# timoblak/sq-recovery

Hardware: NVIDIA B200
Metric: fused SQ implicit-loss fwd+bwd throughput (higher is better)
Workload: dtype f32

## Files before the change

sq_recovery_b200/csrc/sqloss.cu:

```cuda
#include <cuda_runtime.h>
#include <stdint.h>
#include <stdio.h>
#include <string.h>
#include <new>

#include "../../include/sqloss.h"
#ifdef SQ_TIMELINE
__device__ unsigned long long g_bwd_stats[2];
#endif
#if defined(SQ_TIMELINE) && defined(SQ_BWD_STATS)
#define SQ_BWD_HOOK(a) do { const unsigned m_ = __ballot_sync(0xffffffffu, (a)); if ((threadIdx.x & 31) == 0) { \
    atomicAdd(&g_bwd_stats[0], 1ull); atomicAdd(&g_bwd_stats[1], (unsigned long long)__popc(m_)); } } while (0)
#endif
#ifdef SQ_ITEMLOG
__device__ float g_planlog[4 * 65536];
__device__ int g_itemlog[4 * 65536];
#endif
#ifdef SQ_COUNT
__device__ unsigned long long g_count[8];
#define SQ_COUNT_HOOK(i, n) do { if ((threadIdx.x & 31) == 0) atomicAdd(&g_count[i], (unsigned long long)(n)); } while (0)
#else
#define SQ_COUNT_HOOK(i, n) do { } while (0)
#endif
#include "sq_core.cuh"
// ... 123 lines not shown
#define SQ_CLASSES 32
#endif
constexpr int kClasses = SQ_CLASSES;
static_assert(kClasses >= 4 && kClasses <= 32, "the class counters live in one warp's lanes and in the 256-byte control block");
#ifndef SQ_PLAN_THREADS
#define SQ_PLAN_THREADS 512
#endif
constexpr int kPlanThreads = SQ_PLAN_THREADS;
constexpr int kPlanThreadsSmall = 128;
constexpr int kPlanMaxItems = 8192;

struct Control {
    unsigned int ticket;
    unsigned int cursor;
    unsigned int retired;
    unsigned int pad0;
    unsigned int qcount[kClasses];
    unsigned int pad1[64 - 4 - kClasses];
};
static_assert(sizeof(Control) == 256, "Control block is 256 bytes");

constexpr int kRow = 20;
struct Scratch {
    Control* ctl;
    SampleFull* pred;
    SampleFull* tru;
    float* partials;
    double* per_sample;
    double* tv_sum;
    unsigned long long* counts;
    unsigned char* item_class;
    int* queue;
    int queue_cap;
};

inline size_t align_up(size_t v, size_t a) { return (v + a - 1) / a * a; }

size_t scratch_layout(int batch, int n, char* base, Scratch* s) {
    const Layout L = make_layout(n > 0 ? n : 1, 1);
    size_t off = 0;
    auto take = [&](size_t bytes) { size_t o = off; off = align_up(off + bytes, 256); return o; };
    const size_t o_ctl = take(sizeof(Control));
    const size_t o_pred = take(sizeof(SampleFull) * (size_t)batch);
    const size_t o_true = take(sizeof(SampleFull) * (size_t)batch);
    size_t rows_ps = (size_t)L.rows_per_sample;
    const size_t lsq_rows = (size_t)(L.slots + kThreads - 1) / kThreads;
    if (lsq_rows > rows_ps) rows_ps = lsq_rows;
    const size_t o_part = take(sizeof(float) * kRow * rows_ps * (size_t)batch);
    const size_t o_ps = take(sizeof(double) * (size_t)batch);
    const size_t o_tv = take(sizeof(double) * (size_t)batch);
    const size_t o_cnt = take(sizeof(unsigned long long) * 2 * (size_t)batch);
    const size_t cap = (size_t)L.rows_per_sample * (size_t)batch;
    const bool queued = L.rows_per_sample <= kPlanMaxItems && cap < (1u << 30);
    const size_t o_queue = take(queued ? sizeof(int) * kClasses * cap : 0);
    const size_t o_cls = take(queued ? cap : 0);
    if (s) {
        s->ctl = reinterpret_cast<Control*>(base + o_ctl);
        s->pred = reinterpret_cast<SampleFull*>(base + o_pred);
        s->tru = reinterpret_cast<SampleFull*>(base + o_true);
        s->partials = reinterpret_cast<float*>(base + o_part);
        s->per_sample = reinterpret_cast<double*>(base + o_ps);
        s->tv_sum = reinterpret_cast<double*>(base + o_tv);
        s->counts = reinterpret_cast<unsigned long long*>(base + o_cnt);
        s->queue = queued ? reinterpret_cast<int*>(base + o_queue) : nullptr;
        s->item_class = queued ? reinterpret_cast<unsigned char*>(base + o_cls) : nullptr;
        s->queue_cap = (int)cap;
    }
    return off;
}

__device__ __forceinline__ void pdl_wait() {
#ifdef SQ_PDL
    asm volatile("griddepcontrol.wait;" ::: "memory");
#endif
}
__device__ __forceinline__ void pdl_trigger() {
#ifdef SQ_PDL
    asm volatile("griddepcontrol.launch_dependents;");
#endif
}

#ifdef SQ_TIMELINE
__device__ unsigned long long g_plan_ts[16];
__device__ __forceinline__ unsigned long long gtime() { unsigned long long t; asm volatile("mov.u64 %0, %%globaltimer;" : "=l"(t)); return t; }
#endif
constexpr int kSampleWords = (int)(sizeof(Sample) / 4);
constexpr int kFullWords = (int)(sizeof(SampleFull) / 4);
static_assert(sizeof(Sample) % 8 == 0 && sizeof(SampleFull) % 8 == 0, "Sample records must be word-copyable");

__device__ __forceinline__ void load_params(const void* params, int dtype, int b, double* p) {
#pragma unroll
    for (int i = 0; i < 12; ++i)
        p[i] = dtype == SQ_F64 ? static_cast<const double*>(params)[12 * (size_t)b + i]
                               : (double)static_cast<const float*>(params)[12 * (size_t)b + i];
}

__global__ void __launch_bounds__(128)
prep_kernel(const void* params, int dtype, int batch, int clamp, Grid g, SampleFull* out, Control* ctl) {
    __shared__ SampleFull Ssh[4];
    const int warp = threadIdx.x >> 5, lane = threadIdx.x & 31;
    const int b = blockIdx.x * 4 + warp;
    if (blockIdx.x == 0 && threadIdx.x == 0 && ctl) { ctl->ticket = 0u; ctl->cursor = 0u; }
    if (b >= batch) return;
    if (lane == 0) {
        double p[12];
        load_params(params, dtype, b, p);
        prep_sample(p, clamp != 0, g, Ssh[warp]);
    }
    __syncwarp();
    const uint32_t* src = reinterpret_cast<const uint32_t*>(&Ssh[warp]);
    uint32_t* dst = reinterpret_cast<uint32_t*>(out + b);
    for (int w = lane; w < kFullWords; w += 32) dst[w] = src[w];
}

__device__ int group_planes(const Sample& S, const Grid& g, const Layout& L, float bound, int group, float die = 0.f) {
    float cx, cy, hx, hy;
    if (L.patched) {
        const int pw = L.n >> 3, pb = group / pw, pa = group - pb * pw;
        cx = (float)(pa << 3) + 3.5f; cy = (float)(pb << 2) + 1.5f; hx = 3.5f; hy = 1.5f;
    } else {
        xfast_group_footprint(L.n, group, cx, cy, hx, hy);
    }
    return die > 0.f ? footprint_walk(S, g, bound, die, cx, cy, hx, hy) : footprint_planes(S, g, bound, cx, cy, hx, hy);
}

template <int NS, int THREADS>
__global__ void __launch_bounds__(THREADS)
plan_kernel(const void* params_a, const void* params_b, int dtype, int clamp, int heads, Grid g, Layout L, float bound, float die,
            SampleFull* out_a, SampleFull* out_b, Control* ctl, unsigned long long* counts, int* queue, int cap,
            unsigned char* item_class, const float* __restrict__ target, long long tstride, const int* __restrict__ row_off,
            const int* __restrict__ col_off, double* tv_sum) {
    __shared__ SampleFull Ssh[NS];
    __shared__ unsigned char cls[kPlanMaxItems];
    __shared__ unsigned int ccnt[kClasses], cbase[kClasses];
    __shared__ double tv_part[THREADS / 32];
    const int b = blockIdx.x;
#ifdef SQ_TIMELINE
    unsigned long long ts[6]; int nts = 0;
#define SQ_STAMP() do { if (nts < 6) ts[nts++] = gtime(); } while (0)
#else
#define SQ_STAMP() do { } while (0)
#endif
    SQ_STAMP();
    if (threadIdx.x < kClasses) ccnt[threadIdx.x] = 0u;
    if (threadIdx.x == 64) {
        if (b == 0) { ctl->ticket = 0u; ctl->cursor = 0u; }
        if (counts) { counts[2 * b] = 0ull; counts[2 * b + 1] = 0ull; }
    }
    if ((threadIdx.x >> 5) < NS) {
        __shared__ double psh[NS][12];
        const int w = threadIdx.x >> 5, lane = threadIdx.x & 31;
        double* p = psh[w];
        const void* params = w == 0 ? params_a : params_b;
        if (lane < 12)
            p[lane] = dtype == SQ_F64 ? static_cast<const double*>(params)[12 * (size_t)b + lane]
                                      : (double)static_cast<const float*>(params)[12 * (size_t)b + lane];
        __syncwarp();
        double hp_l = 0.0, hrn = 1.0;
        if (heads) {
            double v = 0.0;
            if (lane < 8) { hp_l = (double)(float)(1.0 / (1.0 + exp(-p[lane]))); v = hp_l; }
            else if (lane < 12) {
                hrn = 1.0 / sqrt(p[8] * p[8] + p[9] * p[9] + p[10] * p[10] + p[11] * p[11]);
                v = (double)(float)(p[lane] * hrn);
// ... 26 lines not shown
            int i = t;
            for (; i + 7 * T < npix; i += 8 * T) {
                float v[8];
#pragma unroll
                for (int u = 0; u < 8; ++u) v[u] = pixel(i + u * T);
#pragma unroll
                for (int u = 0; u < 8; u += 2) { acc0 += (double)fabsf(v[u]); acc1 += (double)fabsf(v[u + 1]); }
            }
            {
                float v[8];
#pragma unroll
                for (int u = 0; u < 8; ++u) { const int iu = i + u * T; v[u] = iu < npix ? pixel(iu) : 0.f; }
#pragma unroll
                for (int u = 0; u < 8; u += 2) { acc0 += (double)fabsf(v[u]); acc1 += (double)fabsf(v[u + 1]); }
            }
            double d = acc0 + acc1;
#pragma unroll
            for (int o = 16; o > 0; o >>= 1) d += __shfl_xor_sync(0xffffffffu, d, o);
            if (lane == 0) tv_part[warp] = d;
            SQ_STAMP();
        }
    }
    __syncthreads();
    SQ_STAMP();
    if (tv_sum && threadIdx.x == 0) {
        double d = 0.0;
        for (int w = NS; w < THREADS / 32; ++w) d += tv_part[w];
        tv_sum[b] = d;
    }
    for (int w = threadIdx.x; w < NS * kFullWords; w += THREADS) {
        const int which = w / kFullWords, i = w - which * kFullWords;
        reinterpret_cast<uint32_t*>((which == 0 ? out_a : out_b) + b)[i] = reinterpret_cast<const uint32_t*>(&Ssh[which])[i];
    }
    if (!queue) return;
    const int J = L.rows_per_sample;
    const int max_cost = L.cpt * L.n * NS;
    for (int j = threadIdx.x; j < J; j += THREADS) {
        int c = kClasses - 1;
        int cost = 0;
        for (int k = 0; k < L.cpt; ++k) {
            const int group = j + k * J;
            if (group * 32 >= L.slots) break;
#pragma unroll
            for (int w = 0; w < NS; ++w) cost += group_planes(Ssh[w], g, L, bound, group, NS == 1 ? die : 0.f);
        }
        if (cost > 0) {
            if (kClasses == 8) { c = 0; while (c < kClasses - 2 && (cost << (c + 1)) <= max_cost) ++c; }
            else {
                c = (int)((float)(kClasses / 8) * __log2f((float)max_cost / (float)cost));
                c = c < 0 ? 0 : (c > kClasses - 2 ? kClasses - 2 : c);
            }
        }
#ifdef SQ_ITEMLOG
        if (NS == 1 && b * J + j < 65536) { float* lg = g_planlog + 4 * (b * J + j); lg[0] = (float)c; lg[1] = (float)cost; lg[2] = lg[3] = 0.f; }
#endif
        cls[j] = (unsigned char)c;
        if (item_class) item_class[(size_t)b * J + j] = (unsigned char)c;
        atomicAdd(&ccnt[c], 1u);
    }
    __syncthreads();
    SQ_STAMP();
    if (threadIdx.x < kClasses) {
        const unsigned int c = ccnt[threadIdx.x];
        cbase[threadIdx.x] = c ? atomicAdd(&ctl->qcount[threadIdx.x], c) : 0u;
        ccnt[threadIdx.x] = 0u;
    }
    __syncthreads();
    for (int j = threadIdx.x; j < J; j += THREADS) {
        const int c = cls[j];
        const unsigned int r = atomicAdd(&ccnt[c], 1u);
#ifdef SQ_DEBUG_BOUNDS
        if (c < 0 || c >= kClasses || cbase[c] + r >= (unsigned int)cap || b * J + j >= cap) __trap();
#endif
        queue[(size_t)c * cap + cbase[c] + r] = b * J + j;
    }
#ifdef SQ_TIMELINE
    SQ_STAMP();
    if (b == 7 && (threadIdx.x == 0 || threadIdx.x == 100)) {
        const int o = threadIdx.x == 0 ? 0 : 8;
        for (int i = 0; i < nts; ++i) g_plan_ts[o + i] = ts[i];
        g_plan_ts[o + 7] = nts;
    }
#endif
}

__device__ __forceinline__ float warp_sum(float v) {
#pragma unroll
    for (int o = 16; o > 0; o >>= 1) v += __shfl_xor_sync(0xffffffffu, v, o);
    return v;
}

// ... 94 lines not shown
            for (int w = 0; w < kWarps; ++w) s += red[w][threadIdx.x];
        }
        row[threadIdx.x] = s;
    }
}

__device__ __forceinline__ void load_sample(Sample* dst, const SampleFull* src) {
    const uint32_t* s = reinterpret_cast<const uint32_t*>(src);
    uint32_t* d = reinterpret_cast<uint32_t*>(dst);
    for (int i = threadIdx.x; i < kSampleWords; i += blockDim.x) d[i] = s[i];
}

constexpr int kSampleRegs = (kSampleWords + 31) / 32;
struct SampleFetch {
    uint32_t w[kSampleRegs];
    __device__ __forceinline__ void fetch(const SampleFull* src, int lane) {
        const uint32_t* s = reinterpret_cast<const uint32_t*>(src);
#pragma unroll
        for (int j = 0; j < kSampleRegs; ++j) {
            const int i = lane + 32 * j;
            w[j] = i < kSampleWords ? __ldg(s + i) : 0u;
        }
    }
    __device__ __forceinline__ void commit(Sample* dst, int lane) const {
        uint32_t* d = reinterpret_cast<uint32_t*>(dst);
        __syncwarp();
#pragma unroll
        for (int j = 0; j < kSampleRegs; ++j) {
            const int i = lane + 32 * j;
            if (i < kSampleWords) d[i] = w[j];
        }
        __syncwarp();
    }
};

__device__ __forceinline__ int first_position() {
    return (int)(blockIdx.x * (blockDim.x >> 5) + (threadIdx.x >> 5));
}
__device__ __forceinline__ int next_position(unsigned int* cursor, int lane) {
    int pos = 0;
    if (lane == 0) pos = (int)(atomicAdd(cursor, 1u) + gridDim.x * (blockDim.x >> 5));
    return __shfl_sync(0xffffffffu, pos, 0);
}

struct WorkMap {
    unsigned int excl;
    __device__ __forceinline__ void init(const Control* ctl, int lane) {
        const unsigned int cnt = lane < kClasses ? __ldcg(&ctl->qcount[lane]) : 0u;
        unsigned int incl = cnt;
#pragma unroll
        for (int o = 1; o < kClasses; o <<= 1) {
            const unsigned int t = __shfl_up_sync(0xffffffffu, incl, o);
            if (lane >= o) incl += t;
        }
        excl = incl - cnt;
    }
    __device__ __forceinline__ int item(const int* __restrict__ queue, int cap, int pos, int lane) const {
        if (!queue) return pos;
        const unsigned int m = __ballot_sync(0xffffffffu, lane < kClasses && (unsigned int)pos >= excl);
        const int c = 31 - __clz((int)m);
        const unsigned int start = __shfl_sync(0xffffffffu, excl, c);
#ifdef SQ_DEBUG_BOUNDS
        if (c < 0 || c >= kClasses || (unsigned int)pos - start >= (unsigned int)cap) __trap();
        const int it = __ldg(queue + (size_t)c * cap + ((unsigned int)pos - start));
        if (it < 0 || it >= cap) __trap();
        return it;
// ... 44 lines not shown
        const unsigned int warps = gridDim.x * (blockDim.x >> 5);
        const unsigned int joiners = (unsigned int)total_items < warps ? (unsigned int)total_items : warps;
        const unsigned int before = atomicAdd(&ctl->retired, 1u);
        if (before + 1u == joiners) {
            ctl->retired = 0u;
#pragma unroll
            for (int k = 0; k < kClasses; ++k) ctl->qcount[k] = 0u;
        }
    }
}

#ifdef SQ_TIMELINE
__device__ unsigned long long g_timeline[3 * 8192];
__device__ unsigned int g_classes[kClasses];
#endif
#ifdef SQ_PHASES
__device__ unsigned long long g_phase[8];
#define SQ_PH(i) do { const long long n_ = clock64(); ph[i] += n_ - ph_t; ph_t = n_; } while (0)
#else
#define SQ_PH(i) do { } while (0)
#endif

#ifndef SQ_EARLY_MARGIN
#define SQ_EARLY_MARGIN 0
#endif
constexpr size_t kImplicitBwdSmemPerWarp = (size_t)kBwdPool * 4 * sizeof(float) + 11 * 32 * sizeof(float);
static_assert(kImplicitBwdSmemPerWarp % 32 == 0, "per-warp regions stay 32-byte aligned (BwdQueue::where carries the lane in its low bits)");

template <bool BWD, int THREADS, int MINB, int CPTMAX, bool VJP = false>
__global__ void __launch_bounds__(THREADS, MINB)
implicit_kernel(const SampleFull* __restrict__ samples, Grid g, Layout L, ImplicitParams P, int total_items,
                Control* __restrict__ ctl, const int* __restrict__ queue, int cap,
                const float* __restrict__ target, long long tstride, const int* __restrict__ row_off,
                const int* __restrict__ col_off, float* __restrict__ partials, float* __restrict__ depth_out) {
    __shared__ Sample Ssh[THREADS / 32];
#if SQ_TILE_ALIAS && defined(SQ_BWD_COMPACT)
    static_assert(!BWD || CPTMAX == 1, "SQ_TILE_ALIAS needs one column group per work item");
    static_assert(4 * kBwdPool >= kRedFloats, "pool arrays too small to hold the tile");
    __shared__ __align__(16) float tiles_static[BWD ? 1 : THREADS / 32][kRedFloats];
#else
    __shared__ __align__(16) float tiles_static[THREADS / 32][kRedFloats];
#endif
#ifdef SQ_BWD_COMPACT
    constexpr int kQN = kBwdPool;
    extern __shared__ __align__(32) unsigned char dyn_smem[];
    float* const qbuf = reinterpret_cast<float*>(dyn_smem + (size_t)(threadIdx.x >> 5) * kImplicitBwdSmemPerWarp);
    float* const colinfo_w = qbuf + 4 * kQN;
#endif
#if SQ_TILE_ALIAS && defined(SQ_BWD_COMPACT)
    float* const tile_w = BWD ? qbuf : tiles_static[threadIdx.x >> 5];
#else
    float* const tile_w = tiles_static[threadIdx.x >> 5];
#endif
    static_assert(!VJP || BWD, "the VJP mode is a mode of the fwd+bwd kernel");
    const int warp = threadIdx.x >> 5, lane = threadIdx.x & 31;
    Sample& S = Ssh[warp];
#if defined(SQ_BWD_COMPACT) && !defined(SQ_TABLES_GLOBAL)
    __shared__ __align__(16) double tabs[BWD ? 384 : 130];
    constexpr int kTabRegs = (384 + THREADS - 1) / THREADS;
    double tab_reg[kTabRegs];
    if (BWD) {
#pragma unroll
        for (int r = 0; r < kTabRegs; ++r) {
            const int i = threadIdx.x + r * THREADS;
            tab_reg[r] = i < 128 ? kExp2TabDev[i] : (i < 384 ? kLog2TabDev[i - 128] : 0.0);
        }
    }
    const RefTabs tb{tabs, tabs + 128};
#else
    const RefTabs tb = default_tabs();
#endif
    pdl_wait();
    pdl_trigger();
#ifdef SQ_TIMELINE
    const unsigned long long t_begin = gtime();
    unsigned long long t_last_fetch = t_begin, n_items = 0;
    if (BWD && blockIdx.x == 0 && threadIdx.x < kClasses) g_classes[threadIdx.x] = ctl->qcount[threadIdx.x];
#endif
    WorkPipe wp;
    wp.start(ctl, queue, cap, total_items, true, lane);
#ifdef SQ_PHASES
    long long ph[8] = {0, 0, 0, 0, 0, 0, 0, 0}, ph_t = clock64();
#endif
    {
        SampleFetch pre;
        if (wp.item >= 0) pre.fetch(samples + L.sample_of(wp.item), lane);
#if defined(SQ_BWD_COMPACT) && !defined(SQ_TABLES_GLOBAL)
        if (BWD) {
#pragma unroll
            for (int r = 0; r < kTabRegs; ++r) { const int i = threadIdx.x + r * THREADS; if (i < 384) tabs[i] = tab_reg[r]; }
            __syncthreads();
        }
#endif
        while (wp.item >= 0) {
#ifdef SQ_TIMELINE
            t_last_fetch = gtime(); ++n_items;
#endif
            int b, chunk;
            L.split(wp.item, b, chunk);
#ifdef SQ_ITEMLOG
            const long long il_t0 = clock64(); long long il_walk = 0; int il_q = 0, il_qr = 0;
#endif
            SQ_PH(7);
            pre.commit(&S, lane);
            SQ_COUNT_HOOK(4, 1);

            float loss_sum = 0.f;
            bool folded = false;
            ColIter it;
            it.init(L, chunk, lane);
            float tvs[CPTMAX];
            {
                ColIter pt = it;
#pragma unroll
                for (int k = 0; k < CPTMAX; ++k) {
                    tvs[k] = 0.f;
                    if (target && k < L.cpt) {
                        if (pt.valid(L))
                            tvs[k] = VJP ? __ldg(target + ((size_t)b * g.n + (g.n - 1 - pt.ib)) * g.n + pt.ia)
                                         : __ldg(target + (size_t)b * tstride + row_off[g.n - 1 - pt.ib] + col_off[pt.ia]);
                        pt.next(L);
                    }
                }
            }
#pragma unroll 1
            for (int k = 0; k < L.cpt; ++k) {
#ifdef SQ_EARLY_CLAIM
                if (k == L.cpt - 1 && wp.claim(lane)) pre.fetch(samples + L.sample_of(wp.next), lane);
#endif
                const int ia = it.ia, ib = it.ib;
                const bool valid = it.valid(L);
                const int row = g.n - 1 - ib, col = ia;
                it.next(L);
                float b32[3];
                column_base_f32(S, g, valid ? ia : 0, valid ? ib : 0, b32);
                int c_lo, c_hi;
                column_range(S, g, P.bound, b32, c_lo, c_hi);
                if (!valid) { c_lo = 0; c_hi = -1; }
                const int own_lo = c_hi >= c_lo ? c_lo : g.n;
                warp_range(g.n, c_lo, c_hi);
                if (c_hi < c_lo) {
#ifndef SQ_EARLY_CLAIM
                    if (k == L.cpt - 1 && wp.claim(lane)) pre.fetch(samples + L.sample_of(wp.next), lane);
#endif
                    continue;
                }
                SQ_COUNT_HOOK(5, 1);
                SQ_PH(0);
#ifdef SQ_ITEMLOG
                const long long il_w0 = clock64();
#endif
#if defined(SQ_BWD_COMPACT) && !defined(SQ_NO_STAGED_CLAIM) && !defined(SQ_EARLY_CLAIM) && SQ_EARLY_MARGIN > 0
                const bool early = BWD && k == L.cpt - 1 &&
                                   wp.item_pos + SQ_EARLY_MARGIN * (int)(gridDim.x * (THREADS / 32)) < wp.total;
                if (early) wp.claim_issue(lane);
#else
                const bool early = false;
#endif
                float bh[3], bl[3], cg[11], dxy[2];
                column_base(S, g, valid ? ia : 0, valid ? ib : 0, bh, bl, dxy);
                float depth;
#ifndef SQ_FIXHOIST
#ifdef SQ_BWD_COMPACT
                const int pool = (g.n <= kPoolMaxPlanes && S.cf0 < 1.0f) ? kQN : 0;
                float U = 0.f; int nr = 0, top = pool - 1, head = kNoLink; bool spilled = false;
                unsigned where = (unsigned)__cvta_generic_to_shared(qbuf) | (unsigned)lane;
                asm volatile("" : "+r"(where));
                const BwdQueue qwarp{qbuf, qbuf + kQN, qbuf + 2 * kQN, qbuf + 3 * kQN, pool, lane, where};
                depth = implicit_column<BWD, true, BWD>(S, g, P, bh, bl, c_lo, c_hi, own_lo, cg, &qwarp, &U, &nr, &top, &spilled, &head);
#else
                depth = implicit_column<BWD, true>(S, g, P, bh, bl, c_lo, c_hi, own_lo, cg);
#endif
#else
                if (__any_sync(0xffffffffu, column_zero_possible(S, bh)))
                    depth = implicit_column<BWD, true>(S, g, P, bh, bl, c_lo, c_hi, own_lo, cg);
                else
                    depth = implicit_column<BWD, false>(S, g, P, bh, bl, c_lo, c_hi, own_lo, cg);
#endif
                SQ_PH(1);
#ifdef SQ_ITEMLOG
                il_walk += clock64() - il_w0;
#endif
#ifndef SQ_EARLY_CLAIM
#if defined(SQ_BWD_COMPACT) && !defined(SQ_NO_STAGED_CLAIM)
                const bool staged = BWD && k == L.cpt - 1;
                if (staged) { if (!early) wp.claim_issue(lane); }
                else
#else
                const bool staged = false;
#endif
                if (k == L.cpt - 1 && wp.claim(lane)) pre.fetch(samples + L.sample_of(wp.next), lane);
#endif
#if defined(SQ_BWD_COMPACT)
                if (BWD) {
                    float wsg = 0.f;
                    float tv = tvs[0];
#pragma unroll
                    for (int q = 1; q < CPTMAX; ++q) tv = k == q ? tvs[q] : tv;
                    asm volatile("" : "+f"(tv));
                    if (valid && VJP) {
                        wsg = tv;
                    } else if (valid) {
                        if (depth_out) depth_out[((size_t)b * g.n + row) * g.n + col] = depth;
                        const float diff = depth - tv;
                        loss_sum += fabsf(diff) - fabsf(tv);
                        wsg = diff > 0.f ? 1.f : (diff < 0.f ? -1.f : 0.f);
                    }
                    const int total_r = nr, total = nr + (pool - 1 - top);
                    const bool any_spill = __any_sync(0xffffffffu, spilled && wsg != 0.f);
#ifdef SQ_ITEMLOG
                    il_q += total + (any_spill ? 1000 : 0); il_qr += total_r;
#endif
#ifndef SQ_EARLY_CLAIM
                    if (staged) {
                        wp.claim_lookup(lane);
                        if (total == 0 && wp.claim_finish()) pre.fetch(samples + L.sample_of(wp.next), lane);
                    }
#endif
                    SQ_PH(2);
                    if (total > 0 || any_spill) {
                        Acc acc;
                        float v[kRedStride];
                        if (folded) { tile_get(tile_w, v); array_to_acc(v, acc); } else acc_zero(acc);
                        if (spilled && wsg != 0.f) implicit_fold(acc, cg, wsg, dxy[0], dxy[1]);
                        if (total > 0) {
                            float* ci = colinfo_w;
                            ci[0 * 32 + lane] = bh[0]; ci[1 * 32 + lane] = bh[1]; ci[2 * 32 + lane] = bh[2];
                            ci[3 * 32 + lane] = bl[0]; ci[4 * 32 + lane] = bl[1]; ci[5 * 32 + lane] = bl[2];
                            ci[6 * 32 + lane] = wsg; ci[7 * 32 + lane] = dxy[0]; ci[8 * 32 + lane] = dxy[1];
                            ci[9 * 32 + lane] = U; ci[10 * 32 + lane] = __int_as_float(head);
                            __syncwarp();
                            SQ_COUNT_HOOK(6, total); SQ_COUNT_HOOK(7, total_r);
                            SQ_COUNT_HOOK(3, (total_r + 31) / 32); SQ_COUNT_HOOK(2, (total + 31) / 32);
                            SQ_PH(5);
                            for (int jr = lane; jr < total_r; jr += 32) {
                                const int l_ = entry_lane(qwarp.cf[jr]);
                                queue_refine_entry(S, g.step, P.kl, qwarp, jr,
                                                   f2d(ci[0 * 32 + l_]) + f2d(ci[3 * 32 + l_]), f2d(ci[1 * 32 + l_]) + f2d(ci[4 * 32 + l_]),
                                                   f2d(ci[2 * 32 + l_]) + f2d(ci[5 * 32 + l_]), tb);
                            }
                            __syncwarp();
                            SQ_PH(3);
                            const float tau = P.tl * (float)kLn2;
#ifdef SQ_DEPTH_SHIFT
                            if (!VJP && head != kNoLink) loss_sum = fmaf(wsg * tau * g.inv_n, queue_depth_shift(qwarp, head, U), loss_sum);
#endif
#ifndef SQ_EARLY_CLAIM
                            if (staged && wp.claim_finish()) pre.fetch(samples + L.sample_of(wp.next), lane);
#endif
                            auto dealt = [&](int j, Bwd& bq, float& cfq, float& dx_, float& dy_) {
                                const bool has = j < total;
                                const int at = has ? (j < total_r ? j : kQN - 1 - (j - total_r)) : 0;
                                const float tagged = has ? qwarp.cf[at] : 1.0f, x_ = has ? qwarp.x[at] : 0.0f;
                                const int l_ = entry_lane(tagged);
                                const float cf_ = entry_cf(S, tagged);
                                const float sw_ = has ? queue_suffix_weight(qwarp, at, __float_as_int(ci[10 * 32 + l_]), ci[9 * 32 + l_], tau) : 0.0f;
                                const float cbh[3] = {ci[0 * 32 + l_], ci[1 * 32 + l_], ci[2 * 32 + l_]};
                                const float cbl[3] = {ci[3 * 32 + l_], ci[4 * 32 + l_], ci[5 * 32 + l_]};
                                queue_entry_backward<true>(S, cbh, cbl, cf_, x_, sw_, ci[6 * 32 + l_], has, bq);
                                cfq = cf_; dx_ = ci[7 * 32 + l_]; dy_ = ci[8 * 32 + l_];
                            };
                            int j = lane;
#if SQ_DENSE_ILP == 2
                            for (; j - lane + 32 < total; j += 64) {
                                Bwd b0, b1; float c0, c1, x0, x1, y0, y1;
                                dealt(j, b0, c0, x0, y0);
                                dealt(j + 32, b1, c1, x1, y1);
                                acc_add_point(acc, b0, c0, x0, y0);
                                acc_add_point(acc, b1, c1, x1, y1);
                            }
#endif
                            for (; j - lane < total; j += 32) {
                                Bwd b0; float c0, x0, y0;
                                dealt(j, b0, c0, x0, y0);
                                acc_add_point(acc, b0, c0, x0, y0);
                            }
                            __syncwarp();
                            SQ_PH(4);
                        }
                        acc_to_array(acc, v);
                        v[18] = v[19] = 0.f;
// ... 490 lines not shown
    return sms[dev];
}

int persistent_blocks(int items, int warps_per_block, int min_blocks_per_sm) {
    const int need = (items + warps_per_block - 1) / warps_per_block;
    const int fill = device_sm_count() * min_blocks_per_sm;
    return need < fill ? need : fill;
}

template <auto KERNEL>
cudaError_t opt_in_dyn_smem(size_t dyn) {
    static bool opted[64] = {false};
    int dev = 0;
    cudaGetDevice(&dev);
    if (dev >= 0 && dev < 64 && !opted[dev]) {
        const cudaError_t e = cudaFuncSetAttribute(KERNEL, cudaFuncAttributeMaxDynamicSharedMemorySize, (int)dyn);
        if (e != cudaSuccess) return e;
        opted[dev] = true;
    }
    return cudaSuccess;
}

int launch_prep(const void* params, int dtype, int batch, bool clamp, const Grid& g, SampleFull* out, Control* ctl,
                cudaStream_t st) {
    if (dtype != SQ_F32 && dtype != SQ_F64) return (int)cudaErrorInvalidValue;
    prep_kernel<<<(batch + 3) / 4, 128, 0, st>>>(params, dtype, batch, clamp ? 1 : 0, g, out, ctl);
    return (int)cudaGetLastError();
}

struct PlanTarget { const float* target; long long tstride; const int* row_off; const int* col_off; };

int launch_plan(const void* params_a, const void* params_b, int dtype, int batch, bool clamp, const Grid& g,
                const Layout& L, float bound, const Scratch& s, unsigned long long* counts, unsigned char* item_class,
                const PlanTarget* pt, cudaStream_t st, bool heads = false, float die = 0.f) {
    if (dtype != SQ_F32 && dtype != SQ_F64) return (int)cudaErrorInvalidValue;
    int* queue = L.rows_per_sample <= kPlanMaxItems ? s.queue : nullptr;
    const PlanTarget none{nullptr, 0, nullptr, nullptr};
    const PlanTarget& t = pt ? *pt : none;
    const bool small = batch > 4 * device_sm_count();
    if (params_b) {
        auto k = small ? plan_kernel<2, kPlanThreadsSmall> : plan_kernel<2, kPlanThreads>;
        k<<<batch, small ? kPlanThreadsSmall : kPlanThreads, 0, st>>>(params_a, params_b, dtype, clamp ? 1 : 0, 0, g, L, bound, 0.f, s.tru, s.pred,
                                                                      s.ctl, counts, queue, s.queue_cap, queue ? item_class : nullptr,
                                                                      nullptr, 0, nullptr, nullptr, nullptr);
    } else {
        auto k = small ? plan_kernel<1, kPlanThreadsSmall> : plan_kernel<1, kPlanThreads>;
        k<<<batch, small ? kPlanThreadsSmall : kPlanThreads, 0, st>>>(params_a, nullptr, dtype, clamp ? 1 : 0, heads ? 1 : 0, g, L, bound, die, s.pred,
                                                                      nullptr, s.ctl, counts, queue, s.queue_cap, queue ? item_class : nullptr,
                                                                      t.target, t.tstride, t.row_off, t.col_off, pt ? s.tv_sum : nullptr);
    }
    return (int)cudaGetLastError();
}

}

extern "C" {

const char* sq_version(void) { return "sqloss-b200 0.1 (sm_100a)"; }

const char* sq_error_string(int err) { return cudaGetErrorString((cudaError_t)err); }

int sq_device_sm_count(int device, int* sm_count) {
    return (int)cudaDeviceGetAttribute(sm_count, cudaDevAttrMultiProcessorCount, device);
}

#ifdef SQ_COUNT
int sq_debug_counters(unsigned long long* host_out, int reset) {
    cudaError_t e = cudaMemcpyFromSymbol(host_out, g_count, sizeof(unsigned long long) * 8);
    if (e == cudaSuccess && reset) {
        const unsigned long long zero[8] = {0, 0, 0, 0, 0, 0, 0, 0};
        e = cudaMemcpyToSymbol(g_count, zero, sizeof zero);
    }
    return (int)e;
}
#endif

#ifdef SQ_ITEMLOG
int sq_debug_itemlog(float* plan_out, int* item_out, int n) {
    int rc = (int)cudaMemcpyFromSymbol(plan_out, g_planlog, sizeof(float) * 4 * (size_t)n);
    if (!rc) rc = (int)cudaMemcpyFromSymbol(item_out, g_itemlog, sizeof(int) * 4 * (size_t)n);
    return rc;
}
// ... 3 lines not shown
    int rc = (int)cudaMemcpyFromSymbol(host_out, g_phase, sizeof(unsigned long long) * 8);
    if (!rc && reset) { unsigned long long z[8] = {0, 0, 0, 0, 0, 0, 0, 0}; rc = (int)cudaMemcpyToSymbol(g_phase, z, sizeof z); }
    return rc;
}
#endif
#ifdef SQ_TIMELINE
int sq_debug_timeline(unsigned long long* host_out, int n) {
    return (int)cudaMemcpyFromSymbol(host_out, g_timeline, sizeof(unsigned long long) * 3 * (size_t)n);
}
int sq_debug_bwd(unsigned long long* host_out) {
    return (int)cudaMemcpyFromSymbol(host_out, g_bwd_stats, sizeof(unsigned long long) * 2);
}
int sq_debug_plan(unsigned long long* host_out) {
    return (int)cudaMemcpyFromSymbol(host_out, g_plan_ts, sizeof(unsigned long long) * 16);
}
int sq_debug_classes(unsigned int* host_out) {
    return (int)cudaMemcpyFromSymbol(host_out, g_classes, sizeof(unsigned int) * kClasses);
}
#endif

void sq_profile_events(void* ev_before, void* ev_after) {
    t_ev_before = static_cast<cudaEvent_t>(ev_before);
    t_ev_after = static_cast<cudaEvent_t>(ev_after);
}

size_t sq_scratch_bytes(int batch, int n) {
    if (batch <= 0 || n <= 0) return 0;
    return scratch_layout(batch, n, nullptr, nullptr);
}

int sq_scratch_init(void* scratch, size_t scratch_bytes, sq_stream_t stream) {
    if (!scratch || scratch_bytes < sizeof(Control)) return (int)cudaErrorInvalidValue;
    return (int)cudaMemsetAsync(scratch, 0, sizeof(Control), static_cast<cudaStream_t>(stream));
}

static int implicit_loss_impl(const void* pred, int pred_dtype, int batch, int n, double step, double z0,
                              const float* target, long long target_stride_b, const int* row_off, const int* col_off,
                              float tau, float sharpness, double* loss_out, double* per_sample, void* grad_pred,
                              float* depth_out, void* scratch, size_t scratch_bytes, sq_stream_t stream, bool heads) {
    Scratch s;
    int rc = check_scratch(batch, n, scratch, scratch_bytes, &s);
    if (rc) return rc;
    if (target && (!row_off || !col_off)) return (int)cudaErrorInvalidValue;
    if (grad_pred && !target) return (int)cudaErrorInvalidValue;
    cudaStream_t st = static_cast<cudaStream_t>(stream);
    const Grid g = make_grid(n, step, z0);
    const Layout L = make_layout(n, grad_pred ? SQ_IMPB_CPT : SQ_IMPF_CPT);
    const ImplicitParams P{sharpness * kLog2e, tau * kLog2e, implicit_cull_bound(sharpness * kLog2e), implicit_active_bits(sharpness * kLog2e, n, batch)};
    if (depth_out)
        SQ_TRY(cudaMemsetAsync(depth_out, 0, sizeof(float) * (size_t)batch * n * n, st));
#ifdef SQ_SKIP_COLUMN
    SQ_TRY(cudaMemsetAsync(s.ctl, 0, sizeof(Control), st));
#endif
    const PlanTarget pt{target, target_stride_b, row_off, col_off};
    rc = launch_plan(pred, nullptr, pred_dtype, batch, true, g, L, P.bound, s, nullptr, target ? s.item_class : nullptr,
                     target ? &pt : nullptr, st, heads, SQ_WALK_ESTIMATE ? 32.0f / P.tl : 0.f);
    if (rc) return rc;
    const int items = batch * L.rows_per_sample;
    const int* queue = L.rows_per_sample <= kPlanMaxItems ? s.queue : nullptr;
#ifdef SQ_PDL
    const bool pdl = (t_ev_before == nullptr && t_ev_after == nullptr);
#else
    const bool pdl = false;
#endif
#ifndef SQ_SKIP_COLUMN
    {
        ColumnKernelTimer timer(st);
        if (grad_pred) {
            const int blocks = persistent_blocks(items, SQ_IMPB_THREADS / 32, SQ_IMPB_MINB);
            constexpr size_t dyn = kImplicitBwdSmemPerWarp * (SQ_IMPB_THREADS / 32);
            SQ_TRY((opt_in_dyn_smem<implicit_kernel<true, SQ_IMPB_THREADS, SQ_IMPB_MINB, SQ_IMPB_CPT>>(dyn)));
            SQ_TRY(launch_dependent(implicit_kernel<true, SQ_IMPB_THREADS, SQ_IMPB_MINB, SQ_IMPB_CPT>, blocks, SQ_IMPB_THREADS, dyn, st, pdl,
                                    s.pred, g, L, P, items, s.ctl, queue, s.queue_cap, target, target_stride_b, row_off, col_off,
                                    s.partials, depth_out));
        } else {
            const int blocks = persistent_blocks(items, SQ_IMPF_THREADS / 32, SQ_IMPF_MINB);
            SQ_TRY(launch_dependent(implicit_kernel<false, SQ_IMPF_THREADS, SQ_IMPF_MINB, SQ_IMPF_CPT>, blocks, SQ_IMPF_THREADS, 0, st, pdl,
                                    s.pred, g, L, P, items, s.ctl, queue, s.queue_cap, target, target_stride_b, row_off, col_off,
                                    s.partials, depth_out));
        }
    }
    SQ_TRY(cudaGetLastError());
#endif
#ifndef SQ_SKIP_FINALIZE
    if (target) {
        const double nn = (double)n * n;
        SQ_TRY(launch_dependent(finalize_kernel<FIN_IMPLICIT>, batch, kFinThreads, 0, st, pdl,
                                s.pred, g, batch, L.rows_per_sample, s.partials, 1.0 / nn,
                                -(double)sharpness * (double)tau / (nn * n * (double)batch), pred_dtype, grad_pred, s.per_sample,
                                per_sample, loss_out, &s.ctl->ticket, s.tv_sum, queue ? s.item_class : nullptr));
        SQ_TRY(cudaGetLastError());
    }
#endif
    return 0;
}

int sq_implicit_loss(const void* pred, int pred_dtype, int batch, int n, double step, double z0,
                     const float* target, long long target_stride_b, const int* row_off, const int* col_off,
                     float tau, float sharpness, double* loss_out, double* per_sample, void* grad_pred,
                     float* depth_out, void* scratch, size_t scratch_bytes, sq_stream_t stream) {
    return implicit_loss_impl(pred, pred_dtype, batch, n, step, z0, target, target_stride_b, row_off, col_off, tau, sharpness,
                              loss_out, per_sample, grad_pred, depth_out, scratch, scratch_bytes, stream, false);
}

int sq_implicit_loss_heads(const void* raw_heads, int dtype, int batch, int n, double step, double z0,
                           const float* target, long long target_stride_b, const int* row_off, const int* col_off,
                           float tau, float sharpness, double* loss_out, double* per_sample, void* grad_raw,
                           float* depth_out, void* scratch, size_t scratch_bytes, sq_stream_t stream) {
    return implicit_loss_impl(raw_heads, dtype, batch, n, step, z0, target, target_stride_b, row_off, col_off, tau, sharpness,
                              loss_out, per_sample, grad_raw, depth_out, scratch, scratch_bytes, stream, true);
}

int sq_depth_projection_vjp(const void* pred, int pred_dtype, int batch, int n, double step, double z0,
                            float tau, float sharpness, const float* grad_depth, void* grad_pred,
                            void* scratch, size_t scratch_bytes, sq_stream_t stream) {
    Scratch s;
    int rc = check_scratch(batch, n, scratch, scratch_bytes, &s);
    if (rc) return rc;
    if (!grad_depth || !grad_pred) return (int)cudaErrorInvalidValue;
    cudaStream_t st = static_cast<cudaStream_t>(stream);
    const Grid g = make_grid(n, step, z0);
    const Layout L = make_layout(n, SQ_IMPB_CPT);
    const ImplicitParams P{sharpness * kLog2e, tau * kLog2e, implicit_cull_bound(sharpness * kLog2e), implicit_active_bits(sharpness * kLog2e, n, 1)};
    rc = launch_plan(pred, nullptr, pred_dtype, batch, true, g, L, P.bound, s, nullptr, s.item_class, nullptr, st, false,
                     SQ_WALK_ESTIMATE ? 32.0f / P.tl : 0.f);
    if (rc) return rc;
    const int items = batch * L.rows_per_sample;
    const int* queue = L.rows_per_sample <= kPlanMaxItems ? s.queue : nullptr;
#ifdef SQ_PDL
    const bool pdl = (t_ev_before == nullptr && t_ev_after == nullptr);
#else
    const bool pdl = false;
#endif
    {
        ColumnKernelTimer timer(st);
        const int blocks = persistent_blocks(items, SQ_IMPB_THREADS / 32, SQ_IMPB_MINB);
        constexpr size_t dyn = kImplicitBwdSmemPerWarp * (SQ_IMPB_THREADS / 32);
        SQ_TRY((opt_in_dyn_smem<implicit_kernel<true, SQ_IMPB_THREADS, SQ_IMPB_MINB, SQ_IMPB_CPT, true>>(dyn)));
        SQ_TRY(launch_dependent(implicit_kernel<true, SQ_IMPB_THREADS, SQ_IMPB_MINB, SQ_IMPB_CPT, true>, blocks, SQ_IMPB_THREADS, dyn,
                                st, pdl, s.pred, g, L, P, items, s.ctl, queue, s.queue_cap, grad_depth, 0LL,
                                static_cast<const int*>(nullptr), static_cast<const int*>(nullptr), s.partials,
                                static_cast<float*>(nullptr)));
    }
    SQ_TRY(cudaGetLastError());
    SQ_TRY(launch_dependent(finalize_kernel<FIN_IMPLICIT>, batch, kFinThreads, 0, st, pdl,
                            s.pred, g, batch, L.rows_per_sample, s.partials, 0.0, -(double)sharpness * (double)tau / (double)n,
                            pred_dtype, grad_pred, s.per_sample, static_cast<double*>(nullptr), static_cast<double*>(nullptr),
                            &s.ctl->ticket, static_cast<const double*>(nullptr), queue ? s.item_class : nullptr));
    SQ_TRY(cudaGetLastError());
    return 0;
}

int sq_explicit_loss(const void* true_params, const void* pred, int params_dtype, int batch, int n, double step,
                     double z0, float sharpness, float mult, double* loss_out, double* per_sample, void* grad_pred,
                     void* scratch, size_t scratch_bytes, sq_stream_t stream) {
    Scratch s;
    int rc = check_scratch(batch, n, scratch, scratch_bytes, &s);
    if (rc) return rc;
    if (!true_params || !pred) return (int)cudaErrorInvalidValue;
    cudaStream_t st = static_cast<cudaStream_t>(stream);
    const Grid g = make_grid(n, step, z0);
    const Layout L = make_layout(n, SQ_EXP_CPT);
    const float kl = sharpness * kLog2e, bound = cull_bound_bits(kl, 24.0f);
    rc = launch_plan(true_params, pred, params_dtype, batch, true, g, L, bound, s, nullptr, s.item_class, nullptr, st);
    if (rc) return rc;
    const int items = batch * L.rows_per_sample;
    const int* queue = L.rows_per_sample <= kPlanMaxItems ? s.queue : nullptr;
    const int blocks = persistent_blocks(items, SQ_EXP_THREADS / 32, SQ_EXP_MINB);
    {
        ColumnKernelTimer timer(st);
        if (grad_pred) explicit_kernel<true><<<blocks, SQ_EXP_THREADS, 0, st>>>(s.tru, s.pred, g, L, kl, bound, items, s.ctl, queue, s.queue_cap, s.partials);
        else explicit_kernel<false><<<blocks, SQ_EXP_THREADS, 0, st>>>(s.tru, s.pred, g, L, kl, bound, items, s.ctl, queue, s.queue_cap, s.partials);
    }
    SQ_TRY(cudaGetLastError());
    const double n3 = (double)n * n * n;
// ... 388 lines not shown
```

Baseline: 1360.

## Precompute per-lane column ranges in plan kernel and prefetch them in backward

```diff
diff --git a/sq_recovery_b200/csrc/sqloss.cu b/sq_recovery_b200/csrc/sqloss.cu
--- a/sq_recovery_b200/csrc/sqloss.cu
+++ b/sq_recovery_b200/csrc/sqloss.cu
@@ -179,6 +179,7 @@
     unsigned char* item_class;
     int* queue;
     int queue_cap;
+    uint32_t* ranges;
 };
 
 inline size_t align_up(size_t v, size_t a) { return (v + a - 1) / a * a; }
@@ -201,6 +202,7 @@
     const bool queued = L.rows_per_sample <= kPlanMaxItems && cap < (1u << 30);
     const size_t o_queue = take(queued ? sizeof(int) * kClasses * cap : 0);
     const size_t o_cls = take(queued ? cap : 0);
+    const size_t o_rng = take(sizeof(uint32_t) * 32 * cap);
     if (s) {
         s->ctl = reinterpret_cast<Control*>(base + o_ctl);
         s->pred = reinterpret_cast<SampleFull*>(base + o_pred);
@@ -212,6 +214,7 @@
         s->queue = queued ? reinterpret_cast<int*>(base + o_queue) : nullptr;
         s->item_class = queued ? reinterpret_cast<unsigned char*>(base + o_cls) : nullptr;
         s->queue_cap = (int)cap;
+        s->ranges = reinterpret_cast<uint32_t*>(base + o_rng);
     }
     return off;
 }
@@ -271,12 +274,45 @@
     return die > 0.f ? footprint_walk(S, g, bound, die, cx, cy, hx, hy) : footprint_planes(S, g, bound, cx, cy, hx, hy);
 }
 
+__device__ int plan_item_ranges(const Sample& S, const Grid& g, const Layout& L, float bound, float die, int group,
+                                uint32_t* rec) {
+    const int lane = threadIdx.x & 31;
+    ColIter it;
+    it.init(L, group, lane);
+    const bool valid = it.valid(L);
+    float b32[3];
+    column_base_f32(S, g, valid ? it.ia : 0, valid ? it.ib : 0, b32);
+    int c_lo, c_hi;
+    column_range(S, g, bound, b32, c_lo, c_hi);
+    if (!valid) { c_lo = 0; c_hi = -1; }
+    rec[lane] = (uint32_t)c_lo | ((uint32_t)c_hi << 16);
+    const bool own = c_hi >= c_lo;
+    warp_range(g.n, c_lo, c_hi);
+    if (c_hi < c_lo) return 0;
+    const int planes = c_hi - c_lo + 1;
+    if (!(die > 0.f)) return planes;
+    int cut = planes;
+    if (own) {
+        const float a = fmaf(S.dh[0], S.dh[0], fmaf(S.dh[1], S.dh[1], S.dh[2] * S.dh[2])), nf = (float)(g.n - 1);
+        const float beta = fmaf(S.dh[0], b32[0], fmaf(S.dh[1], b32[1], S.dh[2] * b32[2]));
+        const float gamma = fmaf(b32[0], b32[0], fmaf(b32[1], b32[1], fmaf(b32[2], b32[2], -0.97f)));
+        const float disc = fmaf(beta, beta, -a * gamma);
+        cut = 0;
+        if (disc > 0.f) {
+            const float sq = sqrtf(disc), far_ = fmaxf((-beta - sq) / a, 0.f), near_ = fminf((sq - beta) / a, nf);
+            if (near_ - far_ >= die) cut = (int)(fmaxf(near_ - die - 1.0f, (float)c_lo) - (float)c_lo);
+        }
+    }
+    cut = __reduce_min_sync(0xffffffffu, cut);
+    return cut > 0 ? (planes - cut > 1 ? planes - cut : 1) : planes;
+}
+
 template <int NS, int THREADS>
 __global__ void __launch_bounds__(THREADS)
 plan_kernel(const void* params_a, const void* params_b, int dtype, int clamp, int heads, Grid g, Layout L, float bound, float die,
             SampleFull* out_a, SampleFull* out_b, Control* ctl, unsigned long long* counts, int* queue, int cap,
             unsigned char* item_class, const float* __restrict__ target, long long tstride, const int* __restrict__ row_off,
-            const int* __restrict__ col_off, double* tv_sum) {
+            const int* __restrict__ col_off, double* tv_sum, uint32_t* ranges) {
     __shared__ SampleFull Ssh[NS];
     __shared__ unsigned char cls[kPlanMaxItems];
     __shared__ unsigned int ccnt[kClasses], cbase[kClasses];
@@ -369,18 +405,11 @@
         const int which = w / kFullWords, i = w - which * kFullWords;
         reinterpret_cast<uint32_t*>((which == 0 ? out_a : out_b) + b)[i] = reinterpret_cast<const uint32_t*>(&Ssh[which])[i];
     }
-    if (!queue) return;
+    if (!queue && !ranges) return;
     const int J = L.rows_per_sample;
     const int max_cost = L.cpt * L.n * NS;
-    for (int j = threadIdx.x; j < J; j += THREADS) {
+    auto cost_class = [&](int cost, int j) {
         int c = kClasses - 1;
-        int cost = 0;
-        for (int k = 0; k < L.cpt; ++k) {
-            const int group = j + k * J;
-            if (group * 32 >= L.slots) break;
-#pragma unroll
-            for (int w = 0; w < NS; ++w) cost += group_planes(Ssh[w], g, L, bound, group, NS == 1 ? die : 0.f);
-        }
         if (cost > 0) {
             if (kClasses == 8) { c = 0; while (c < kClasses - 2 && (cost << (c + 1)) <= max_cost) ++c; }
             else {
@@ -391,9 +420,41 @@
 #ifdef SQ_ITEMLOG
         if (NS == 1 && b * J + j < 65536) { float* lg = g_planlog + 4 * (b * J + j); lg[0] = (float)c; lg[1] = (float)cost; lg[2] = lg[3] = 0.f; }
 #endif
-        cls[j] = (unsigned char)c;
-        if (item_class) item_class[(size_t)b * J + j] = (unsigned char)c;
-        atomicAdd(&ccnt[c], 1u);
+        return c;
+    };
+    if (queue) {
+        for (int j = threadIdx.x; j < J; j += THREADS) {
+            int cost = 0;
+            for (int k = 0; k < L.cpt; ++k) {
+                const int group = j + k * J;
+                if (group * 32 >= L.slots) break;
+#pragma unroll
+                for (int w = 0; w < NS; ++w) cost += group_planes(Ssh[w], g, L, bound, group, NS == 1 ? die : 0.f);
+            }
+            const int c = cost_class(cost, j);
+            cls[j] = (unsigned char)c;
+            if (!ranges) {
+                if (item_class) item_class[(size_t)b * J + j] = (unsigned char)c;
+                atomicAdd(&ccnt[c], 1u);
+            }
+        }
+    }
+    if (NS == 1 && ranges) {
+        if (queue) __syncthreads();
+        const int warp = threadIdx.x >> 5, lane = threadIdx.x & 31;
+        for (int j = warp; j < J; j += THREADS / 32) {
+            if (queue && cls[j] == kClasses - 1) continue;
+            const size_t item = (size_t)b * J + j;
+            const int cost = plan_item_ranges(Ssh[0], g, L, bound, die, j, ranges + 32 * item);
+            if (queue && lane == 0) cls[j] = (unsigned char)cost_class(cost, j);
+        }
+        if (!queue) return;
+        __syncthreads();
+        for (int j = threadIdx.x; j < J; j += THREADS) {
+            const int c = cls[j];
+            if (item_class) item_class[(size_t)b * J + j] = (unsigned char)c;
+            atomicAdd(&ccnt[c], 1u);
+        }
     }
     __syncthreads();
     SQ_STAMP();
@@ -554,6 +615,12 @@
         }
         __syncwarp();
     }
+    __device__ __forceinline__ static void fetch_ranges(uint32_t* dst, const uint32_t* ranges, int item, int lane) {
+        asm volatile("cp.async.ca.shared.global [%0], [%1], 4;"
+                     :: "r"((unsigned)__cvta_generic_to_shared(dst + lane)), "l"(ranges + 32 * (size_t)item + lane) : "memory");
+        asm volatile("cp.async.commit_group;" ::: "memory");
+    }
+    __device__ __forceinline__ static void ranges_wait() { asm volatile("cp.async.wait_all;" ::: "memory"); }
 };
 
 __device__ __forceinline__ int first_position() {
@@ -664,7 +731,8 @@
 implicit_kernel(const SampleFull* __restrict__ samples, Grid g, Layout L, ImplicitParams P, int total_items,
                 Control* __restrict__ ctl, const int* __restrict__ queue, int cap,
                 const float* __restrict__ target, long long tstride, const int* __restrict__ row_off,
-                const int* __restrict__ col_off, float* __restrict__ partials, float* __restrict__ depth_out) {
+                const int* __restrict__ col_off, float* __restrict__ partials, float* __restrict__ depth_out,
+                const uint32_t* __restrict__ ranges) {
     __shared__ Sample Ssh[THREADS / 32];
 #if SQ_TILE_ALIAS && defined(SQ_BWD_COMPACT)
     static_assert(!BWD || CPTMAX == 1, "SQ_TILE_ALIAS needs one column group per work item");
@@ -685,8 +753,11 @@
     float* const tile_w = tiles_static[threadIdx.x >> 5];
 #endif
     static_assert(!VJP || BWD, "the VJP mode is a mode of the fwd+bwd kernel");
+    static_assert(!BWD || CPTMAX == 1, "the plan kernel's range records cover one column group per work item");
     const int warp = threadIdx.x >> 5, lane = threadIdx.x & 31;
     Sample& S = Ssh[warp];
+    __shared__ uint32_t ranges_sh[THREADS / 32][32];
+    uint32_t* const ranges_w = ranges_sh[warp];
 #if defined(SQ_BWD_COMPACT) && !defined(SQ_TABLES_GLOBAL)
     __shared__ __align__(16) double tabs[BWD ? 384 : 130];
     constexpr int kTabRegs = (384 + THREADS - 1) / THREADS;
@@ -716,7 +787,13 @@
 #endif
     {
         SampleFetch pre;
-        if (wp.item >= 0) pre.fetch(samples + L.sample_of(wp.item), lane);
+        auto fetch = [&](int item) {
+            pre.fetch(samples + L.sample_of(item), lane);
+#ifdef SQ_BWD_COMPACT
+            if (BWD) SampleFetch::fetch_ranges(ranges_w, ranges, item, lane);
+#endif
+        };
+        if (wp.item >= 0) fetch(wp.item);
 #if defined(SQ_BWD_COMPACT) && !defined(SQ_TABLES_GLOBAL)
         if (BWD) {
 #pragma unroll
@@ -734,6 +811,9 @@
             const long long il_t0 = clock64(); long long il_walk = 0; int il_q = 0, il_qr = 0;
 #endif
             SQ_PH(7);
+#ifdef SQ_BWD_COMPACT
+            if (BWD) SampleFetch::ranges_wait();
+#endif
             pre.commit(&S, lane);
             SQ_COUNT_HOOK(4, 1);
 
@@ -758,22 +838,31 @@
 #pragma unroll 1
             for (int k = 0; k < L.cpt; ++k) {
 #ifdef SQ_EARLY_CLAIM
-                if (k == L.cpt - 1 && wp.claim(lane)) pre.fetch(samples + L.sample_of(wp.next), lane);
+                if (k == L.cpt - 1 && wp.claim(lane)) fetch(wp.next);
 #endif
                 const int ia = it.ia, ib = it.ib;
                 const bool valid = it.valid(L);
                 const int row = g.n - 1 - ib, col = ia;
                 it.next(L);
-                float b32[3];
-                column_base_f32(S, g, valid ? ia : 0, valid ? ib : 0, b32);
                 int c_lo, c_hi;
-                column_range(S, g, P.bound, b32, c_lo, c_hi);
-                if (!valid) { c_lo = 0; c_hi = -1; }
+#ifdef SQ_BWD_COMPACT
+                if (BWD) {
+                    const uint32_t rec = ranges_w[lane];
+                    c_lo = (int)(rec & 0xffffu);
+                    c_hi = (int)rec >> 16;
+                } else
+#endif
+                {
+                    float b32[3];
+                    column_base_f32(S, g, valid ? ia : 0, valid ? ib : 0, b32);
+                    column_range(S, g, P.bound, b32, c_lo, c_hi);
+                    if (!valid) { c_lo = 0; c_hi = -1; }
+                }
                 const int own_lo = c_hi >= c_lo ? c_lo : g.n;
                 warp_range(g.n, c_lo, c_hi);
                 if (c_hi < c_lo) {
 #ifndef SQ_EARLY_CLAIM
-                    if (k == L.cpt - 1 && wp.claim(lane)) pre.fetch(samples + L.sample_of(wp.next), lane);
+                    if (k == L.cpt - 1 && wp.claim(lane)) fetch(wp.next);
 #endif
                     continue;
                 }
@@ -821,7 +910,7 @@
 #else
                 const bool staged = false;
 #endif
-                if (k == L.cpt - 1 && wp.claim(lane)) pre.fetch(samples + L.sample_of(wp.next), lane);
+                if (k == L.cpt - 1 && wp.claim(lane)) fetch(wp.next);
 #endif
 #if defined(SQ_BWD_COMPACT)
                 if (BWD) {
@@ -846,7 +935,7 @@
 #ifndef SQ_EARLY_CLAIM
                     if (staged) {
                         wp.claim_lookup(lane);
-                        if (total == 0 && wp.claim_finish()) pre.fetch(samples + L.sample_of(wp.next), lane);
+                        if (total == 0 && wp.claim_finish()) fetch(wp.next);
                     }
 #endif
                     SQ_PH(2);
@@ -878,7 +967,7 @@
                             if (!VJP && head != kNoLink) loss_sum = fmaf(wsg * tau * g.inv_n, queue_depth_shift(qwarp, head, U), loss_sum);
 #endif
 #ifndef SQ_EARLY_CLAIM
-                            if (staged && wp.claim_finish()) pre.fetch(samples + L.sample_of(wp.next), lane);
+                            if (staged && wp.claim_finish()) fetch(wp.next);
 #endif
                             auto dealt = [&](int j, Bwd& bq, float& cfq, float& dx_, float& dy_) {
                                 const bool has = j < total;
@@ -1435,8 +1524,9 @@
 
 int launch_plan(const void* params_a, const void* params_b, int dtype, int batch, bool clamp, const Grid& g,
                 const Layout& L, float bound, const Scratch& s, unsigned long long* counts, unsigned char* item_class,
-                const PlanTarget* pt, cudaStream_t st, bool heads = false, float die = 0.f) {
+                const PlanTarget* pt, cudaStream_t st, bool heads = false, float die = 0.f, bool ranges = false) {
     if (dtype != SQ_F32 && dtype != SQ_F64) return (int)cudaErrorInvalidValue;
+    if (ranges && (params_b || L.cpt != 1 || L.n > 32767)) return (int)cudaErrorInvalidValue;
     int* queue = L.rows_per_sample <= kPlanMaxItems ? s.queue : nullptr;
     const PlanTarget none{nullptr, 0, nullptr, nullptr};
     const PlanTarget& t = pt ? *pt : none;
@@ -1445,12 +1535,13 @@
         auto k = small ? plan_kernel<2, kPlanThreadsSmall> : plan_kernel<2, kPlanThreads>;
         k<<<batch, small ? kPlanThreadsSmall : kPlanThreads, 0, st>>>(params_a, params_b, dtype, clamp ? 1 : 0, 0, g, L, bound, 0.f, s.tru, s.pred,
                                                                       s.ctl, counts, queue, s.queue_cap, queue ? item_class : nullptr,
-                                                                      nullptr, 0, nullptr, nullptr, nullptr);
+                                                                      nullptr, 0, nullptr, nullptr, nullptr, nullptr);
     } else {
         auto k = small ? plan_kernel<1, kPlanThreadsSmall> : plan_kernel<1, kPlanThreads>;
         k<<<batch, small ? kPlanThreadsSmall : kPlanThreads, 0, st>>>(params_a, nullptr, dtype, clamp ? 1 : 0, heads ? 1 : 0, g, L, bound, die, s.pred,
                                                                       nullptr, s.ctl, counts, queue, s.queue_cap, queue ? item_class : nullptr,
-                                                                      t.target, t.tstride, t.row_off, t.col_off, pt ? s.tv_sum : nullptr);
+                                                                      t.target, t.tstride, t.row_off, t.col_off, pt ? s.tv_sum : nullptr,
+                                                                      ranges ? s.ranges : nullptr);
     }
     return (int)cudaGetLastError();
 }
@@ -1520,6 +1611,15 @@
 int sq_scratch_init(void* scratch, size_t scratch_bytes, sq_stream_t stream) {
     if (!scratch || scratch_bytes < sizeof(Control)) return (int)cudaErrorInvalidValue;
     return (int)cudaMemsetAsync(scratch, 0, sizeof(Control), static_cast<cudaStream_t>(stream));
+}
+
+int sq_debug_plan_records(int batch, int n, size_t* item_class_off, size_t* ranges_off) {
+    if (batch <= 0 || n <= 0 || !item_class_off || !ranges_off) return (int)cudaErrorInvalidValue;
+    Scratch s;
+    scratch_layout(batch, n, nullptr, &s);
+    *item_class_off = s.item_class ? (size_t)(uintptr_t)s.item_class : SIZE_MAX;
+    *ranges_off = (size_t)(uintptr_t)s.ranges;
+    return 0;
 }
 
 static int implicit_loss_impl(const void* pred, int pred_dtype, int batch, int n, double step, double z0,
@@ -1542,7 +1642,7 @@
 #endif
     const PlanTarget pt{target, target_stride_b, row_off, col_off};
     rc = launch_plan(pred, nullptr, pred_dtype, batch, true, g, L, P.bound, s, nullptr, target ? s.item_class : nullptr,
-                     target ? &pt : nullptr, st, heads, SQ_WALK_ESTIMATE ? 32.0f / P.tl : 0.f);
+                     target ? &pt : nullptr, st, heads, SQ_WALK_ESTIMATE ? 32.0f / P.tl : 0.f, grad_pred != nullptr);
     if (rc) return rc;
     const int items = batch * L.rows_per_sample;
     const int* queue = L.rows_per_sample <= kPlanMaxItems ? s.queue : nullptr;
@@ -1560,12 +1660,12 @@
             SQ_TRY((opt_in_dyn_smem<implicit_kernel<true, SQ_IMPB_THREADS, SQ_IMPB_MINB, SQ_IMPB_CPT>>(dyn)));
             SQ_TRY(launch_dependent(implicit_kernel<true, SQ_IMPB_THREADS, SQ_IMPB_MINB, SQ_IMPB_CPT>, blocks, SQ_IMPB_THREADS, dyn, st, pdl,
                                     s.pred, g, L, P, items, s.ctl, queue, s.queue_cap, target, target_stride_b, row_off, col_off,
-                                    s.partials, depth_out));
+                                    s.partials, depth_out, static_cast<const uint32_t*>(s.ranges)));
         } else {
             const int blocks = persistent_blocks(items, SQ_IMPF_THREADS / 32, SQ_IMPF_MINB);
             SQ_TRY(launch_dependent(implicit_kernel<false, SQ_IMPF_THREADS, SQ_IMPF_MINB, SQ_IMPF_CPT>, blocks, SQ_IMPF_THREADS, 0, st, pdl,
                                     s.pred, g, L, P, items, s.ctl, queue, s.queue_cap, target, target_stride_b, row_off, col_off,
-                                    s.partials, depth_out));
+                                    s.partials, depth_out, static_cast<const uint32_t*>(nullptr)));
         }
     }
     SQ_TRY(cudaGetLastError());
@@ -1611,7 +1711,7 @@
     const Layout L = make_layout(n, SQ_IMPB_CPT);
     const ImplicitParams P{sharpness * kLog2e, tau * kLog2e, implicit_cull_bound(sharpness * kLog2e), implicit_active_bits(sharpness * kLog2e, n, 1)};
     rc = launch_plan(pred, nullptr, pred_dtype, batch, true, g, L, P.bound, s, nullptr, s.item_class, nullptr, st, false,
-                     SQ_WALK_ESTIMATE ? 32.0f / P.tl : 0.f);
+                     SQ_WALK_ESTIMATE ? 32.0f / P.tl : 0.f, true);
     if (rc) return rc;
     const int items = batch * L.rows_per_sample;
     const int* queue = L.rows_per_sample <= kPlanMaxItems ? s.queue : nullptr;
@@ -1628,7 +1728,7 @@
         SQ_TRY(launch_dependent(implicit_kernel<true, SQ_IMPB_THREADS, SQ_IMPB_MINB, SQ_IMPB_CPT, true>, blocks, SQ_IMPB_THREADS, dyn,
                                 st, pdl, s.pred, g, L, P, items, s.ctl, queue, s.queue_cap, grad_depth, 0LL,
                                 static_cast<const int*>(nullptr), static_cast<const int*>(nullptr), s.partials,
-                                static_cast<float*>(nullptr)));
+                                static_cast<float*>(nullptr), static_cast<const uint32_t*>(s.ranges)));
     }
     SQ_TRY(cudaGetLastError());
     SQ_TRY(launch_dependent(finalize_kernel<FIN_IMPLICIT>, batch, kFinThreads, 0, st, pdl,
```

Result: slower. 1302 (median of 6 runs) (-4.3%).
